# bempt/uda_aerial_semantic_segmentation_research

Measured on AMD Instinct MI355X. Metric: training images/sec at 512x512, higher is better.
Workload: dtype fp32

## Files before the change

include/udaseg.h:

```cpp
#ifndef UDASEG_H
#define UDASEG_H

#include <stddef.h>
#include <stdint.h>

#ifdef __cplusplus
extern "C" {
#endif

#define UDASEG_OK 0
#define UDASEG_E_BADARG (-1)
#define UDASEG_E_UNSUPPORTED (-2)
#define UDASEG_E_WORKSPACE (-3)
#define UDASEG_E_HIP (-4)

#define UDASEG_ACT_NONE 0
#define UDASEG_ACT_LEAKY 1

int udaseg_version(void);
#define UDASEG_OPT_GENERIC_GATHER 0
#define UDASEG_OPT_F32_SPLIT 1
#define UDASEG_OPT_WGRAD_GENERIC 2
#define UDASEG_OPT_F32_HALO 3
#define UDASEG_OPT_F3_CFG 4
#define UDASEG_OPT_F3_WS 5
#define UDASEG_OPT_F3_SIGNS 6
#define UDASEG_OPT_IGEMM_TILE 7
#define UDASEG_OPT_IGEMM_X3 8
#define UDASEG_OPT_NO_FOLD 9
#define UDASEG_OPT_WGRAD_X3_BLOCKS 10
#define UDASEG_OPT_WGRAD_BLOCKS 11
#define UDASEG_OPT_WGRAD_NO_XCD 12
#define UDASEG_OPT_WGRAD_X3 13
#define UDASEG_OPT_NO_WGRAD_HALO 14
#define UDASEG_OPT_WGRAD_F3_BLOCKS 15
#define UDASEG_OPT_WGRAD_HALO_BLOCKS 16
#define UDASEG_OPT_WGRAD_DEEP_BLOCKS 17
#define UDASEG_OPT_WGRAD_DB 18
#define UDASEG_OPT_REDUCE_BLOCKS 19
#define UDASEG_OPT_BN_APPLY_PT 20
#define UDASEG_OPT_GEMM_1X1_TILE 21
#define UDASEG_OPT_GEMM_1X1 22
#define UDASEG_OPT_GEMM_1X1_MAXM 23
#define UDASEG_OPT_NO_STREAM 24
#define UDASEG_OPT_HALO_CFG 25
#define UDASEG_OPT_NO_HALO 26
#define UDASEG_OPT_NO_HALO_S2 27
#define UDASEG_OPT_HALO_W16 28
#define UDASEG_OPT_HALO_DEEP 29
#define UDASEG_OPT_HALO_S2_CK 30
#define UDASEG_OPT_UP_CFG 31
#define UDASEG_OPT_WGRAD_UP_BLOCKS 32
#define UDASEG_OPT_COUNT 33
int udaseg_set_option(int key, int value);
int udaseg_get_option(int key);
int udaseg_option_count(void);
const char* udaseg_option_name(int key);
int udaseg_option_epoch(void);
const char* udaseg_last_error(void);
int udaseg_device_count(void);
int udaseg_memset_async(void* ptr, int value, size_t bytes, void* stream);
int udaseg_stream_wait(void* waiter_stream, void* signal_stream);

typedef struct {
  int n, hi, wi, ci;
  int ho, wo, co;
  int kh, kw, stride, pad;
} udaseg_conv_desc;


int udaseg_conv2d_fwd(const udaseg_conv_desc* d, const float* x, const float* w, const float* bias, float* y,
                      int act, float slope, int accumulate, void* stream);
int udaseg_conv2d_fwd_bnstats(const udaseg_conv_desc* d, const float* x, const float* w, const float* bias, float* y,
                              double* stats, void* stream);
int udaseg_conv2d_fwd_fused(const udaseg_conv_desc* d, const float* x, const float* w, const float* bias,
                            const float* residual, float* y, int act, float slope, void* stream);
int udaseg_conv2d_fwd_bf16(const udaseg_conv_desc* d, const void* x, const void* w, const float* bias, const void* residual,
                           void* y, int out_f32, int act, float slope, double* stats, void* stream);
int udaseg_conv2d_dgrad_bf16(const udaseg_conv_desc* d, const void* dy, const void* w_t, void* dx, int accumulate,
                             void* stream);
int udaseg_conv2d_wgrad_bf16(const udaseg_conv_desc* d, const void* x, const void* dy, float* dw, int accumulate, void* stream);
int udaseg_conv2d_dgrad(const udaseg_conv_desc* d, const float* dy, const float* w_t, float* dx, int accumulate,
                        void* stream);
int udaseg_conv2d_dgrad_bnreduce_ok(const udaseg_conv_desc* d);
int udaseg_conv2d_dgrad_bnreduce(const udaseg_conv_desc* d, const float* dy, const float* w_t, float* dx, const float* prev_y,
                                 const float* save_mean, const float* save_rstd, const float* gamma, const float* beta, int act,
                                 float slope, double* bsums, void* stream);
int udaseg_conv2d_dgrad_bnreduce_bf16_ok(const udaseg_conv_desc* d);
int udaseg_conv2d_dgrad_bnreduce_bf16(const udaseg_conv_desc* d, const void* dy, const void* w_t, void* dx, const void* prev_y,
                                      const float* save_mean, const float* save_rstd, const float* gamma, const float* beta,
                                      int act, float slope, double* bsums, void* stream);
int udaseg_conv2d_wgrad(const udaseg_conv_desc* d, const float* x, const float* dy, float* dw, int accumulate,
                        void* stream);
int udaseg_conv2d_fwd_upcat(const udaseg_conv_desc* d, const float* a, const float* skip, int ca, const float* w,
                            const float* bias, float* y, int act, float slope, double* stats, void* stream);
int udaseg_conv2d_fwd_upcat_bf16(const udaseg_conv_desc* d, const void* a, const void* skip, int ca, const void* w,
                                 const float* bias, void* y, int act, float slope, double* stats, void* stream);
int udaseg_conv2d_dgrad_split(const udaseg_conv_desc* d, const float* dy, const float* w_t, float* dx_a, float* dx_b, int ca,
                              void* stream);
int udaseg_conv2d_dgrad_split_bf16(const udaseg_conv_desc* d, const void* dy, const void* w_t, void* dx_a, void* dx_b, int ca,
                                   void* stream);
int udaseg_conv2d_wgrad_part(const udaseg_conv_desc* d, const float* src, int src_c, int c_off, int up, const float* dy,
                             float* dw, int accumulate, void* stream);
int udaseg_conv2d_wgrad_part_bf16(const udaseg_conv_desc* d, const void* src, int src_c, int c_off, int up, const void* dy,
                                  float* dw, int accumulate, void* stream);
int udaseg_pack_dgrad_weights(const udaseg_conv_desc* d, const float* w, float* w_t, void* stream);
// ... 227 lines not shown
```

uda_aerial_semantic_segmentation_research_amd/_lib.py:

```python
import ctypes as C
import os

_HERE = os.path.dirname(os.path.abspath(__file__))
LIB_PATH = os.environ.get("UDASEG_LIB", os.path.join(_HERE, "libudaseg_hip.so"))

ACT_NONE = 0
ACT_LEAKY = 1


class ConvDesc(C.Structure):
    _fields_ = [(k, C.c_int) for k in ("n", "hi", "wi", "ci", "ho", "wo", "co", "kh", "kw", "stride", "pad")]


_P = C.c_void_p
_I = C.c_int
_L = C.c_int64
_F = C.c_float
_D = C.POINTER(ConvDesc)

SIGNATURES = {
    "udaseg_version": (_I, []),
    "udaseg_set_option": (_I, [_I, _I]),
    "udaseg_get_option": (_I, [_I]),
    "udaseg_option_count": (_I, []),
# ... 92 lines not shown
    "udaseg_bn_bwd_apply_recompute_bf16": (_I, [_P, _P, _P, _P, _P, _P, _P, _P, _P, _P, _P, _L, _I, _I, _F, _P]),
    "udaseg_conv2d_wgrad_halo_bf16_ok": (_I, [_D, _I]),
    "udaseg_conv2d_wgrad_halo_bf16": (_I, [_D, _P, _P, _I, _P, _P, _P]),
    "udaseg_conv2d_wgrad_bnin_bf16": (_I, [_D, _P, _P, _P, _I, _F, _P, _P, _I, _P]),
    "udaseg_frag_elems": (_L, [_I, _I, _I]),
    "udaseg_set_stats_scratch": (_I, [_P, C.c_size_t]),
    "udaseg_pack_frag_batched_bf16": (_I, [_P, _P, _P, _P, _I, _P]),
    "udaseg_conv_frag_ok": (_I, [_D, _I, _I]),
    "udaseg_conv_frag_preferred": (_I, [_D, _I, _I]),
    "udaseg_conv2d_fwd_frag_bf16": (_I, [_D, _P, _P, _I, _P, _P, _P, _P, _I, _F, _P, _I, _I, _F, _P, _P]),
    "udaseg_conv2d_dgrad_frag_bf16": (_I, [_D, _P, _P, _P, _P, _I, _P, _P, _P, _P, _P, _I, _F, _P, _I, _P]),
    "udaseg_pack_frag_batched_f32x3": (_I, [_P, _P, _P, _P, _I, _P]),
    "udaseg_conv2d_wgrad_halo_f32x3_ok": (_I, [_D, _I]),
    "udaseg_conv2d_wgrad_halo_f32x3": (_I, [_D, _P, _P, _I, _P, _P, _P]),
    "udaseg_conv_f32x3_ok": (_I, [_D, _I, _I]),
    "udaseg_f32x3_force_config": (_I, [_I]),
    "udaseg_conv_f32x3_preferred": (_I, [_D, _I, _I]),
    "udaseg_conv2d_fwd_f32x3": (_I, [_D, _P, _P, _I, _P, _P, _P, _I, _F, _P, _P]),
    "udaseg_conv2d_fwd_f32x3_bnin_ok": (_I, [_D, _I]),
    "udaseg_conv2d_fwd_f32x3_bnin_writes": (_I, [_D]),
    "udaseg_conv2d_fwd_f32x3_bnin": (_I, [_D, _P, _I, _P, _P, _I, _F, _P, _P, _P, _P, _I, _F, _P, _P]),
    "udaseg_conv2d_wgrad_bnin_ok": (_I, [_D, _I]),
    "udaseg_conv2d_wgrad_bnin": (_I, [_D, _P, _I, _P, _P, _I, _F, _P, _P, _I, _P]),
    "udaseg_conv2d_dgrad_f32x3": (_I, [_D, _P, _P, _P, _P, _I, _P, _P, _P, _P, _P, _I, _F, _P, _I, _P]),
    "udaseg_conv_up_f32x3_ok": (_I, [_D, _I]),
    "udaseg_pack_up_batched_f32x3": (_I, [_P, _P, _P, _P, _I, _P]),
    "udaseg_conv2d_fwd_up_f32x3": (_I, [_D, _P, _I, _P, _P, _I, _P, _P]),
    "udaseg_conv2d_dgrad_up_f32x3": (_I, [_D, _P, _I, _P, _P, _P, _P, _P, _P, _P, _I, _F, _P, _I, _P]),
    "udaseg_up_f32x3_force_config": (_I, [_I]),
    "udaseg_conv2d_wgrad_up_f32x3_ok": (_I, [_D, _I]),
    "udaseg_conv2d_wgrad_up_f32x3": (_I, [_D, _P, _I, _P, _P, _P]),
    "udaseg_conv2d_wgrad_halo_slice_f32x3": (_I, [_D, _P, _P, _P, _I, _I, _P]),
    "udaseg_wgrad_up_set_blocks": (_I, [_I]),
    "udaseg_conv_stem_f32x3_ok": (_I, [_D]),
    "udaseg_conv2d_fwd_stem_f32x3": (_I, [_D, _P, _P, _P, _P, _P]),
    "udaseg_conv_n16_f32x3_ok": (_I, [_D, _I]),
    "udaseg_conv2d_fwd_n16_f32x3": (_I, [_D, _P, _P, _P, _I, _F, _P, _P, _P, _P]),
    "udaseg_conv2d_dgrad_n16_f32x3": (_I, [_D, _P, _P, _P, _P, _P, _P, _P, _P, _I, _F, _P, _P]),
    "udaseg_set_workspace": (_I, [_P, C.c_size_t]),
    "udaseg_workspace_bytes": (C.c_size_t, [_D]),
    "udaseg_debug_set_timeline": (_I, [_P, _I]),
    "udaseg_fill_f32": (_I, [_P, _L, _F, _P]),
    "udaseg_axpy_f32": (_I, [_P, _P, _L, _F, _P]),
    "udaseg_add_i64": (_I, [_P, _L, _L, _P]),
    "udaseg_prof_enable": (_I, [_I]),
    "udaseg_prof_reset": (_I, []),
    "udaseg_prof_read": (_I, [_I, C.POINTER(C.c_double), C.POINTER(C.c_double), C.POINTER(C.c_int64)]),
    "udaseg_prof_kernel_count": (_I, []),
    "udaseg_prof_kernel_name": (C.c_char_p, [_I]),
    "udaseg_prof_kernel_read": (_I, [_I, C.POINTER(C.c_double), C.POINTER(C.c_double), C.POINTER(C.c_int64)]),
    "udaseg_prof_records": (_I, [_I, _I, C.POINTER(C.c_double), C.POINTER(C.c_double), C.POINTER(C.c_int), C.POINTER(C.c_int)]),
}

OPTIONS = {"GENERIC_GATHER": 0, "F32_SPLIT": 1, "WGRAD_GENERIC": 2, "F32_HALO": 3, "F3_CFG": 4, "F3_WS": 5, "F3_SIGNS": 6, "IGEMM_TILE": 7, "IGEMM_X3": 8, "NO_FOLD": 9, "WGRAD_X3_BLOCKS": 10, "WGRAD_BLOCKS": 11, "WGRAD_NO_XCD": 12, "WGRAD_X3": 13, "NO_WGRAD_HALO": 14, "WGRAD_F3_BLOCKS": 15, "WGRAD_HALO_BLOCKS": 16, "WGRAD_DEEP_BLOCKS": 17, "WGRAD_DB": 18, "REDUCE_BLOCKS": 19, "BN_APPLY_PT": 20, "GEMM_1X1_TILE": 21, "GEMM_1X1": 22, "GEMM_1X1_MAXM": 23, "NO_STREAM": 24, "HALO_CFG": 25, "NO_HALO": 26, "NO_HALO_S2": 27, "HALO_W16": 28, "HALO_DEEP": 29, "HALO_S2_CK": 30, "UP_CFG": 31, "WGRAD_UP_BLOCKS": 32}

_lib = None


def load():
    global _lib
    if _lib is not None:
        return _lib
    if not os.path.exists(LIB_PATH):
        raise RuntimeError(
            f"{LIB_PATH} not found: the HIP extension is not built. Run `python -c \"import __graft_entry__ as g; "
            f"g.build()\"` (or `make -C {os.path.join(_HERE, 'csrc')}`). There is no CPU fallback.")
    lib = C.CDLL(LIB_PATH)
    for name, (res, args) in SIGNATURES.items():
        fn = getattr(lib, name)
        fn.restype = res
        fn.argtypes = args
    _lib = lib
    return lib


def check(rc, what=""):
    if rc != 0:
        msg = load().udaseg_last_error().decode(errors="replace")
        raise RuntimeError(f"libudaseg_hip {what} failed (rc={rc}): {msg}")


def require_gpu():
    lib = load()
    if lib.udaseg_device_count() < 1:
        raise RuntimeError("libudaseg_hip: no HIP device visible; this path has no CPU fallback")
    return lib
```

uda_aerial_semantic_segmentation_research_amd/csrc/api.hip:

```cpp
#include <string.h>
#include <mutex>
#include <vector>

#include "common.h"
#include "options.h"

namespace udaseg {

static thread_local char g_err[512] = "";

void set_error(const char* fmt, ...) {
  va_list ap;
  va_start(ap, fmt);
  vsnprintf(g_err, sizeof(g_err), fmt, ap);
  va_end(ap);
}

int hip_fail(hipError_t e, const char* what) {
  set_error("%s: %s", what, hipGetErrorString(e));
  return UDASEG_E_HIP;
}

struct ProfRec {
  hipEvent_t a, b;
// ... 191 lines not shown
    if (e != hipSuccess) return hip_fail(e, "hipEventSynchronize(prof)");
    float t = 0.f;
    e = hipEventElapsedTime(&t, r.a, r.b);
    if (e != hipSuccess) return hip_fail(e, "hipEventElapsedTime(prof)");
    ms[n] = t;
    flops[n] = r.flops;
    kind[n] = r.kind;
    const int v[11] = {r.d.n, r.d.hi, r.d.wi, r.d.ci, r.d.ho, r.d.wo, r.d.co, r.d.kh, r.d.kw, r.d.stride, r.d.pad};
    for (int i = 0; i < 11; ++i) desc11[n * 11 + i] = v[i];
    ++n;
  }
  return n;
}

namespace udaseg {
enum { K_INT, K_FLAG, K_OFF0 };
struct OptRow {
  const char* env;
  int kind, dflt;
};
static const OptRow g_opt_rows[UDASEG_OPT_COUNT] = {
     {"UDASEG_IGEMM_GENERIC", K_INT, 0},
     {"UDASEG_F32_SPLIT", K_OFF0, 1},
     {"UDASEG_WGRAD_GENERIC", K_INT, 0},
     {"UDASEG_F32_SPLIT", K_OFF0, 1},
     {"UDASEG_F3_CFG", K_INT, 0},
     {"UDASEG_F3_WS", K_OFF0, 1},
     {"UDASEG_F3_SIGNS", K_OFF0, 1},
     {"UDASEG_IGEMM_TILE", K_INT, 0},
     {"UDASEG_IGEMM_X3", K_INT, 1},
     {"UDASEG_NO_FOLD", K_FLAG, 0},
     {"UDASEG_WGRAD_X3_BLOCKS", K_INT, 1024},
     {"UDASEG_WGRAD_BLOCKS", K_INT, 0},
     {"UDASEG_WGRAD_NO_XCD", K_FLAG, 0},
     {"UDASEG_WGRAD_X3", K_OFF0, 1},
     {"UDASEG_NO_WGRAD_HALO", K_FLAG, 0},
     {"UDASEG_WGRAD_F3_BLOCKS", K_INT, 120},
     {"UDASEG_WGRAD_HALO_BLOCKS", K_INT, 96},
     {"UDASEG_WGRAD_DEEP_BLOCKS", K_INT, 0},
     {"UDASEG_WGRAD_DB", K_INT, 1},
     {"UDASEG_REDUCE_BLOCKS", K_INT, 0},
     {"UDASEG_BN_APPLY_PT", K_INT, 4},
     {"UDASEG_GEMM_1X1_TILE", K_INT, 0},
     {"UDASEG_GEMM_1X1", K_OFF0, 1},
     {"UDASEG_GEMM_1X1_MAXM", K_INT, 73728},
     {"UDASEG_NO_STREAM", K_FLAG, 0},
     {"UDASEG_HALO_CFG", K_INT, 0},
     {"UDASEG_NO_HALO", K_FLAG, 0},
     {"UDASEG_NO_HALO_S2", K_FLAG, 0},
     {"UDASEG_HALO_W16", K_INT, 6},
     {"UDASEG_HALO_DEEP", K_OFF0, 1},
     {"UDASEG_HALO_S2_CK", K_INT, 64},
     {"UDASEG_UP_CFG", K_INT, 0},
     {"UDASEG_WGRAD_UP_BLOCKS", K_INT, 0}};
int g_opt_val[UDASEG_OPT_COUNT];
static int g_opt_default[UDASEG_OPT_COUNT];
std::atomic<bool> g_opt_ready{false};
static std::atomic<int> g_opt_epoch{0};
static std::mutex g_opt_mutex;
void opt_init() {
  std::lock_guard<std::mutex> lk(g_opt_mutex);
  if (g_opt_ready.load(std::memory_order_relaxed)) return;
  for (int k = 0; k < UDASEG_OPT_COUNT; ++k) {
    const OptRow& r = g_opt_rows[k];
    const char* e = getenv(r.env);
    int v = r.dflt;
    if (r.kind == K_INT) v = e ? atoi(e) : r.dflt;
    else if (r.kind == K_FLAG) v = e != nullptr ? 1 : 0;
    else v = (e && atoi(e) == 0) ? 0 : 1;
    g_opt_default[k] = g_opt_val[k] = v;
  }
  g_opt_ready.store(true, std::memory_order_release);
}
}

extern "C" int udaseg_set_option(int key, int value) {
  UDASEG_CHECK_ARG(key >= 0 && key < UDASEG_OPT_COUNT, "set_option: unknown key %d (0 .. %d)", key, UDASEG_OPT_COUNT - 1);
  UDASEG_CHECK_ARG(value >= -1, "set_option: value must be >= 0, or -1 for the default");
  udaseg::opt_get(key);
  std::lock_guard<std::mutex> lk(udaseg::g_opt_mutex);
  udaseg::g_opt_val[key] = value < 0 ? udaseg::g_opt_default[key] : value;
  if (key == UDASEG_OPT_GENERIC_GATHER)
    udaseg::g_opt_val[UDASEG_OPT_WGRAD_GENERIC] = value < 0 ? udaseg::g_opt_default[UDASEG_OPT_WGRAD_GENERIC] : value;
  udaseg::g_opt_epoch.fetch_add(1);
  return UDASEG_OK;
}

extern "C" int udaseg_get_option(int key) {
  if (key < 0 || key >= UDASEG_OPT_COUNT) return -1;
  return udaseg::opt_get(key);
}

extern "C" int udaseg_option_count(void) { return UDASEG_OPT_COUNT; }
extern "C" const char* udaseg_option_name(int key) { return key >= 0 && key < UDASEG_OPT_COUNT ? udaseg::g_opt_rows[key].env : ""; }
extern "C" int udaseg_option_epoch(void) { return udaseg::g_opt_epoch.load(); }

extern "C" int udaseg_prof_kernel_count(void) { return g_nkernels; }
extern "C" const char* udaseg_prof_kernel_name(int kid) { return kname(kid); }

extern "C" int udaseg_prof_kernel_read(int kid, double* total_ms, double* total_flops, int64_t* launches) {
  UDASEG_CHECK_ARG(kid >= 0 && kid < g_nkernels && total_ms && total_flops && launches, "prof_kernel_read: bad arguments");
  double ms = 0.0, fl = 0.0;
  for (auto& r : g_krecs[kid]) {
    hipError_t e = hipEventSynchronize(r.b);
    if (e != hipSuccess) return hip_fail(e, "hipEventSynchronize(kprof)");
    float t = 0.f;
    e = hipEventElapsedTime(&t, r.a, r.b);
// ... 10 lines not shown
```

uda_aerial_semantic_segmentation_research_amd/csrc/common.h:

```cpp
#pragma once
#include <stdlib.h>
#include <hip/hip_runtime.h>
#include <stdint.h>
#include <stdio.h>
#include <stdarg.h>
#include <atomic>

#include "../../include/udaseg.h"
#include "options.h"

namespace udaseg {

void set_error(const char* fmt, ...);
int hip_fail(hipError_t e, const char* what);

#define UDASEG_CHECK_ARG(cond, ...)                 \
  do {                                              \
    if (!(cond)) {                                  \
      ::udaseg::set_error(__VA_ARGS__);             \
      return UDASEG_E_BADARG;                       \
    }                                               \
  } while (0)

#define UDASEG_LAUNCH_CHECK(what)                          \
// ... 110 lines not shown
void* workspace_ptr(size_t* bytes);

constexpr int CHSUM_REPLICAS = 16;
constexpr int CHSUM_DIRECT_BLOCKS = 32;
static __global__ void fold_replicas_kernel(const float* __restrict__ rep, int c, float* __restrict__ out, int accumulate) {
  const int i = blockIdx.x * blockDim.x + threadIdx.x;
  if (i >= c) return;
  float s = 0.f;
#pragma unroll
  for (int r = 0; r < CHSUM_REPLICAS; ++r) s += rep[(size_t)r * c + i];
  out[i] = accumulate ? out[i] + s : s;
}

struct StreamShape {
  int bs;
  int grid;
  int c4;
};

static inline StreamShape stream_shape(int64_t n4, int c4, int max_blocks = 2048, int per_thread = 4) {
  StreamShape s;
  s.c4 = c4;
  int unit;
  if (c4 <= 256) {
    s.bs = (256 / c4) * c4;
    unit = 1;
  } else {
    s.bs = 256;
    unit = (c4 + 255) / 256;
    while ((unit * 256) % c4 != 0) ++unit;
  }
  int64_t want = (n4 + (int64_t)s.bs * per_thread - 1) / ((int64_t)s.bs * per_thread);
  if (want > max_blocks) want = max_blocks;
  if (want < 1) want = 1;
  s.grid = (int)(((want + unit - 1) / unit) * unit);
  while ((int64_t)s.grid * s.bs < c4) s.grid += unit;
  return s;
}


static inline int apply_per_thread() {
  const int v = opt_get(UDASEG_OPT_BN_APPLY_PT);
  return (v < 1 || v > 256) ? 4 : v;
}

bool small_conv_applicable(int k, int stride, int pad, int ci_gather, int co_out);
int launch_small_conv(const float* x, const float* w, const float* bias, float* y, int n, int h, int wd, int ci, int co,
                      int flip, int accumulate, int act, float slope, double* stats, const float* residual, hipStream_t s,
                      int up = 0);
bool small_wgrad_applicable(int k, int stride, int pad, int ci, int co, int ntiles);
int launch_small_wgrad(const float* x, const float* dy, float* dw, int n, int h, int wd, int ci, int co, int accumulate,
                       hipStream_t s, int up = 0, const float* in_scale = nullptr, const float* in_shift = nullptr,
                       int in_act = 0, float in_slope = 0.f);

constexpr int PROF_NKERNELS = 24;
int kprof_id(const char* rocprof_symbol);
hipEvent_t kprof_begin(hipStream_t s);
void kprof_end(int kid, hipEvent_t a, hipStream_t s, double flops);
struct KTimer {
  std::atomic<int>* kid;
  hipStream_t s;
  hipEvent_t ev;
  double work;
  KTimer(std::atomic<int>* k, const char* rocprof_symbol, hipStream_t st, double w) : kid(k), s(st), work(w) {
    if (*kid < 0) *kid = kprof_id(rocprof_symbol);
    ev = kprof_begin(s);
  }
  ~KTimer() { kprof_end(*kid, ev, s, work); }
};
void prof_begin(int family, hipStream_t s);
void prof_suspend(int on);
void prof_end(int family, hipStream_t s, double flops, int kind, const udaseg_conv_desc* d);

}
```

uda_aerial_semantic_segmentation_research_amd/csrc/conv_small.hip:

```cpp
#include "common.h"

namespace udaseg {

constexpr int ST = 16;
constexpr int SH = ST + 2;

constexpr int MAX_DEVICES = 16;
static void* g_workspace[MAX_DEVICES] = {};
static size_t g_workspace_bytes[MAX_DEVICES] = {};
static int current_device() {
  int dev = 0;
  if (hipGetDevice(&dev) != hipSuccess || dev < 0 || dev >= MAX_DEVICES) return -1;
  return dev;
}

struct SmallArgs {
  const float* x;
  const float* w;
  const float* bias;
  float* y;
  int n, h, wd, ci, co;
  const float* residual;
  double* stats;
  int flip;
// ... 418 lines not shown
    hipLaunchKernelGGL((conv3x3_small_kernel<2, 1>), dim3(small_grid(a.ntiles, 3)), block, 0, s, a);
    kprof_end(5, ev, s, fl);
  } else if (G == 1 && T == 2) {
    hipLaunchKernelGGL((conv3x3_small_kernel<1, 2>), dim3(small_grid(a.ntiles, 6)), block, 0, s, a);
    kprof_end(6, ev, s, fl);
  } else {
    set_error("small conv: unsupported channel groups G=%d T=%d", G, T);
    return UDASEG_E_UNSUPPORTED;
  }
  UDASEG_LAUNCH_CHECK("conv3x3_small launch");
  return UDASEG_OK;
}

bool small_wgrad_applicable(int k, int stride, int pad, int ci, int co, int ntiles) {
  if (!small_conv_applicable(k, stride, pad, ci, co)) return false;
  const int G = (ci + 15) / 16, T = (co + 15) / 16;
  const size_t need = (size_t)small_grid(ntiles, 2) * (16 * T) * 9 * (16 * G) * sizeof(float);
  const int dev = current_device();
  return dev >= 0 && g_workspace[dev] != nullptr && g_workspace_bytes[dev] >= need;
}

int launch_small_wgrad(const float* x, const float* dy, float* dw, int n, int h, int wd, int ci, int co, int accumulate,
                       hipStream_t s, int up, const float* in_scale, const float* in_shift, int in_act, float in_slope) {
  SmallWgradArgs a = {};
  a.up = up;
  a.in_scale = in_scale; a.in_shift = in_shift; a.in_act = in_act; a.in_slope = in_slope;
  const int dev = current_device();
  if (dev < 0 || g_workspace[dev] == nullptr) {
    set_error("small wgrad: no workspace bound to the current device");
    return UDASEG_E_WORKSPACE;
  }
  a.x = x; a.dy = dy; a.partial = static_cast<float*>(g_workspace[dev]);
  a.n = n; a.h = h; a.w = wd; a.ci = ci; a.co = co;
  a.tiles_x = cdiv(wd, ST); a.tiles_y = cdiv(h, ST); a.ntiles = n * a.tiles_x * a.tiles_y;
  const int G = cdiv(ci, 16), T = cdiv(co, 16);
  const int grid = small_grid(a.ntiles, 2);
  dim3 block(256);
  const double fl = 2.0 * (double)n * h * wd * co * 9.0 * ci;
  hipEvent_t ev = kprof_begin(s);
  if (G == 1 && T == 1) {
    hipLaunchKernelGGL((conv3x3_small_wgrad_kernel<1, 1>), dim3(grid), block, 0, s, a);
    kprof_end(9, ev, s, fl);
  } else if (G == 2 && T == 1) {
    hipLaunchKernelGGL((conv3x3_small_wgrad_kernel<2, 1>), dim3(grid), block, 0, s, a);
    kprof_end(10, ev, s, fl);
  } else if (G == 1 && T == 2) {
    hipLaunchKernelGGL((conv3x3_small_wgrad_kernel<1, 2>), dim3(grid), block, 0, s, a);
    kprof_end(11, ev, s, fl);
  } else {
    set_error("small wgrad: unsupported channel groups G=%d T=%d", G, T);
    return UDASEG_E_UNSUPPORTED;
  }
  UDASEG_LAUNCH_CHECK("conv3x3_small_wgrad launch");
  const int out = 16 * T * 9 * 16 * G;
  if (!accumulate) {
    hipError_t e = hipMemsetAsync(dw, 0, (size_t)co * 9 * ci * sizeof(float), s);
    if (e != hipSuccess) return hip_fail(e, "hipMemsetAsync(small wgrad)");
  }
  hipLaunchKernelGGL(small_wgrad_fold_kernel, dim3(cdiv(out, 256), FOLD_SLICES), dim3(256), 0, s, a.partial, grid, 16 * T, 16 * G,
                     co, ci, dw);
  UDASEG_LAUNCH_CHECK("small_wgrad_fold launch");
  return UDASEG_OK;
}

}

namespace udaseg {
void* workspace_ptr(size_t* bytes) {
  const int dev = current_device();
  if (dev < 0 || g_workspace[dev] == nullptr) {
    if (bytes) *bytes = 0;
    return nullptr;
  }
  if (bytes) *bytes = g_workspace_bytes[dev];
  return g_workspace[dev];
}
}

extern "C" size_t udaseg_workspace_bytes(const udaseg_conv_desc* d) {
  if (!d || d->kh != d->kw || !udaseg::small_conv_applicable(d->kh, d->stride, d->pad, d->ci, d->co)) return 0;
  const int G = (d->ci + 15) / 16, T = (d->co + 15) / 16;
  const int ntiles = d->n * udaseg::cdiv(d->hi, udaseg::ST) * udaseg::cdiv(d->wi, udaseg::ST);
  return (size_t)udaseg::small_grid(ntiles, 2) * (16 * T) * 9 * (16 * G) * sizeof(float);
}

extern "C" int udaseg_set_workspace(void* ptr, size_t bytes) {
  const int dev = udaseg::current_device();
  UDASEG_CHECK_ARG(dev >= 0, "set_workspace: no current HIP device (or more than %d devices)", udaseg::MAX_DEVICES);
  udaseg::g_workspace[dev] = ptr;
  udaseg::g_workspace_bytes[dev] = ptr ? bytes : 0;
  return UDASEG_OK;
}
```

uda_aerial_semantic_segmentation_research_amd/csrc/conv_wgrad.hip:

```cpp
#include <stdlib.h>

#include <type_traits>

#include "common.h"
#include "halo_common.h"

namespace udaseg {

struct WgradArgs {
  const void* x;
  const void* dy;
  float* dw;
  int hi, wi, ci, ho, wo, co;
  int kw, stride, pad;
  int M, J;
  int kchunk;
  int use_atomic;
  float inv_ci, inv_kw, inv_wo, inv_ho;
  int row_uniform;
  unsigned x_bytes, dy_bytes;
  int ci_full, c_off, J_ld, up;
  const float* in_scale;
  const float* in_shift;
  int in_act;
// ... 866 lines not shown
}


}

using namespace udaseg;

static bool wgrad_x3_on() {
  return udaseg::opt_get(UDASEG_OPT_WGRAD_X3) != 0 && udaseg::f32_split_enabled();
}

static int conv2d_wgrad_impl(const udaseg_conv_desc* d, const void* x, int src_c, int c_off, int up, const void* dy, float* dw,
                             int accumulate, void* stream, int bf16, const float* in_scale = nullptr, const float* in_shift = nullptr,
                             int in_act = UDASEG_ACT_NONE, float in_slope = 0.f) {
  UDASEG_CHECK_ARG(d && x && dy && dw, "conv2d_wgrad: NULL pointer");
  const int g = bf16 ? 8 : 4;
  UDASEG_CHECK_ARG(d->ci % g == 0 && d->co % g == 0 && d->ci > 0 && d->co > 0, "conv2d_wgrad: channels must be multiples of %d", g);
  UDASEG_CHECK_ARG(d->kh > 0 && d->kw > 0 && d->stride >= 1 && d->pad >= 0, "conv2d_wgrad: bad kernel/stride");
  UDASEG_CHECK_ARG(d->n > 0 && d->hi > 0 && d->wi > 0 && d->ho > 0 && d->wo > 0, "conv2d_wgrad: non-positive extent");
  UDASEG_CHECK_ARG(d->ho == (d->hi + 2 * d->pad - d->kh) / d->stride + 1 && d->wo == (d->wi + 2 * d->pad - d->kw) / d->stride + 1,
                   "conv2d_wgrad: output extent %dx%d inconsistent with input %dx%d k%d s%d p%d", d->ho, d->wo, d->hi, d->wi,
                   d->kh, d->stride, d->pad);
  UDASEG_CHECK_ARG((long long)d->n * d->hi * d->wi * d->ci < (1LL << 31) && (long long)d->n * d->ho * d->wo * d->co < (1LL << 31),
                   "conv2d_wgrad: tensor exceeds 2^31 elements");
  UDASEG_CHECK_ARG(src_c > 0 && src_c % g == 0 && c_off >= 0 && c_off % g == 0 && c_off + src_c <= d->ci,
                   "conv2d_wgrad_part: channel slice [%d, %d) of %d", c_off, c_off + src_c, d->ci);
  UDASEG_CHECK_ARG(!up || (d->stride == 1 && d->hi % 2 == 0 && d->wi % 2 == 0), "conv2d_wgrad_part: an up-sampled source needs stride 1 and even extents");
  const bool whole = src_c == d->ci;
  UDASEG_CHECK_ARG(whole || accumulate, "conv2d_wgrad_part: a channel slice of dW must be accumulated onto a caller-zeroed gradient");
  WgradArgs a = {};
  a.x = x; a.dy = dy; a.dw = dw;
  a.hi = d->hi; a.wi = d->wi; a.ci = src_c; a.ho = d->ho; a.wo = d->wo; a.co = d->co;
  a.kw = d->kw; a.stride = d->stride; a.pad = d->pad;
  a.M = d->n * d->ho * d->wo;
  a.J = d->kh * d->kw * src_c;
  a.ci_full = d->ci; a.c_off = c_off; a.J_ld = d->kh * d->kw * d->ci; a.up = up;
  a.in_scale = in_scale; a.in_shift = in_shift; a.in_act = in_act; a.in_slope = in_slope;
  a.inv_ci = 1.0f / src_c; a.inv_kw = 1.0f / d->kw; a.inv_wo = 1.0f / d->wo; a.inv_ho = 1.0f / d->ho;
  if (d->kh == 1 && d->kw == 1 && d->stride == 1 && d->pad == 0 && !up) {
    a.hi = 1; a.wi = a.M; a.ho = 1; a.wo = a.M;
    a.inv_wo = 1.0f / (float)a.M; a.inv_ho = 1.0f;
  }
  hipStream_t st = as_stream(stream);
  prof_begin(1, st);
  int rc;
  udaseg_conv_desc dp = *d;
  dp.ci = src_c;
  if (bf16)
    rc = d->co >= 128 ? launch_wgrad<128, 64, 2, 2>(a, accumulate, st, true)
       : d->co > 32   ? launch_wgrad<64, 64, 2, 2>(a, accumulate, st, true)
                      : launch_wgrad<32, 128, 1, 4>(a, accumulate, st, true);
  else if (whole && d->kh == d->kw &&
           small_wgrad_applicable(d->kh, d->stride, d->pad, d->ci, d->co, d->n * cdiv(d->hi, 16) * cdiv(d->wi, 16)))
    rc = launch_small_wgrad(static_cast<const float*>(x), static_cast<const float*>(dy), dw, d->n, d->hi, d->wi, d->ci, d->co,
                            accumulate, st, up);
  else if (d->co > 32 && src_c % 8 == 0 && d->co % 8 == 0 && wgrad_x3_on()) rc = launch_wgrad_x3<64, 64, 2, 2>(a, accumulate, st);
  else if (d->co > 32) rc = launch_wgrad<64, 64, 2, 2>(a, accumulate, st);
  else rc = launch_wgrad<32, 128, 1, 4>(a, accumulate, st);
  prof_end(1, st, udaseg_conv_flops(&dp), 2, &dp);
  return rc;
}

extern "C" int udaseg_conv2d_wgrad(const udaseg_conv_desc* d, const float* x, const float* dy, float* dw,
                                   int accumulate, void* stream) {
  UDASEG_CHECK_ARG(d != nullptr, "conv2d_wgrad: NULL desc");
  return conv2d_wgrad_impl(d, x, d->ci, 0, 0, dy, dw, accumulate, stream, 0);
}

extern "C" int udaseg_conv2d_wgrad_bf16(const udaseg_conv_desc* d, const void* x, const void* dy, float* dw, int accumulate,
                                        void* stream) {
  UDASEG_CHECK_ARG(d != nullptr, "conv2d_wgrad_bf16: NULL desc");
  return conv2d_wgrad_impl(d, x, d->ci, 0, 0, dy, dw, accumulate, stream, 1);
}

extern "C" int udaseg_conv2d_wgrad_bnin_bf16(const udaseg_conv_desc* d, const void* x, const float* in_scale, const float* in_shift,
                                             int in_act, float in_slope, const void* dy, float* dw, int accumulate, void* stream) {
  UDASEG_CHECK_ARG(d != nullptr && in_scale != nullptr && in_shift != nullptr, "conv2d_wgrad_bnin_bf16: NULL desc / scale / shift");
  return conv2d_wgrad_impl(d, x, d->ci, 0, 0, dy, dw, accumulate, stream, 1, in_scale, in_shift, in_act, in_slope);
}

namespace udaseg {
bool wgrad_h2_applicable(const udaseg_conv_desc* d, int up_ca, bool f32);
int launch_wgrad_h2(const udaseg_conv_desc* d, const void* x, const void* x2, int up_ca, const void* dy, float* dw, bool f32, hipStream_t s,
                    const float* in_scale = nullptr, const float* in_shift = nullptr, int in_act = 0, float in_slope = 0.f,
                    int ldw = 0, int dw_coff = 0);
static bool wgrad_halo_off(bool f32) {
  const bool off = opt_get(UDASEG_OPT_NO_WGRAD_HALO) != 0;
  return f32 ? (off || !f32_halo_enabled()) : off;
}
}

extern "C" int udaseg_conv2d_wgrad_bnin_ok(const udaseg_conv_desc* d, int up) {
  if (!d || d->kh != 3 || d->kw != 3 || d->stride != 1 || d->pad != 1 || d->n <= 0 || d->hi <= 0 || d->wi <= 0 || d->ci % 8 != 0 ||
      d->co % 4 != 0)
    return 0;
  if (small_wgrad_applicable(d->kh, d->stride, d->pad, d->ci, d->co, d->n * cdiv(d->hi, 16) * cdiv(d->wi, 16))) return 1;
  return !up && !wgrad_halo_off(true) && wgrad_h2_applicable(d, 0, true) ? 1 : 0;
}

extern "C" int udaseg_conv2d_wgrad_bnin(const udaseg_conv_desc* d, const float* x, int up, const float* in_scale, const float* in_shift,
                                        int in_act, float in_slope, const float* dy, float* dw, int accumulate, void* stream) {
  UDASEG_CHECK_ARG(d && x && in_scale && in_shift && dy && dw, "conv2d_wgrad_bnin: NULL pointer");
  UDASEG_CHECK_ARG(in_act == UDASEG_ACT_NONE || in_act == UDASEG_ACT_LEAKY, "conv2d_wgrad_bnin: unknown activation %d", in_act);
  UDASEG_CHECK_ARG(d->ho == d->hi && d->wo == d->wi, "conv2d_wgrad_bnin: stride-1 'same' convolutions only");
  UDASEG_CHECK_ARG(!up || (d->hi % 2 == 0 && d->wi % 2 == 0), "conv2d_wgrad_bnin: an up-sampled source needs even extents");
  if (!udaseg_conv2d_wgrad_bnin_ok(d, up)) {
    set_error("conv2d_wgrad_bnin: geometry not supported (ask udaseg_conv2d_wgrad_bnin_ok)");
    return UDASEG_E_UNSUPPORTED;
  }
  hipStream_t st = as_stream(stream);
  const bool small = small_wgrad_applicable(d->kh, d->stride, d->pad, d->ci, d->co, d->n * cdiv(d->hi, 16) * cdiv(d->wi, 16));
  if (!small && !accumulate) {
    hipError_t e = hipMemsetAsync(dw, 0, (size_t)d->co * 9 * d->ci * sizeof(float), st);
    if (e != hipSuccess) return hip_fail(e, "hipMemsetAsync(dw)");
  }
  prof_begin(1, st);
  int rc;
  if (small) {
    rc = launch_small_wgrad(x, dy, dw, d->n, d->hi, d->wi, d->ci, d->co, accumulate, st, up, in_scale, in_shift, in_act, in_slope);
  } else {
    rc = launch_wgrad_h2(d, x, nullptr, 0, dy, dw, true, st, in_scale, in_shift, in_act, in_slope);
  }
  prof_end(1, st, udaseg_conv_flops(d), 2, d);
  return rc;
}

extern "C" int udaseg_conv2d_wgrad_halo_bf16_ok(const udaseg_conv_desc* d, int up_ca) {
  return d != nullptr && !wgrad_halo_off(false) && wgrad_h2_applicable(d, up_ca, false) ? 1 : 0;
}

extern "C" int udaseg_conv2d_wgrad_halo_bf16(const udaseg_conv_desc* d, const void* x, const void* skip, int up_ca, const void* dy,
                                             float* dw, void* stream) {
  UDASEG_CHECK_ARG(d && x && dy && dw, "conv2d_wgrad_halo_bf16: NULL pointer");
  UDASEG_CHECK_ARG(d->n > 0 && d->hi > 0 && d->wi > 0 && d->ho == d->hi && d->wo == d->wi, "conv2d_wgrad_halo_bf16: bad extents");
  UDASEG_CHECK_ARG(up_ca == 0 ? skip == nullptr : skip != nullptr, "conv2d_wgrad_halo_bf16: up_ca and skip come together");
  if (!udaseg_conv2d_wgrad_halo_bf16_ok(d, up_ca)) {
    set_error("conv2d_wgrad_halo_bf16: geometry not supported (ask udaseg_conv2d_wgrad_halo_bf16_ok first)");
    return UDASEG_E_UNSUPPORTED;
  }
  hipStream_t st = as_stream(stream);
  prof_begin(1, st);
  const int rc = launch_wgrad_h2(d, x, skip, up_ca, dy, dw, false, st);
  prof_end(1, st, udaseg_conv_flops(d), 2, d);
  return rc;
}

extern "C" int udaseg_conv2d_wgrad_halo_f32x3_ok(const udaseg_conv_desc* d, int up_ca) {
  return d != nullptr && !wgrad_halo_off(true) && wgrad_h2_applicable(d, up_ca, true) ? 1 : 0;
}

extern "C" int udaseg_conv2d_wgrad_halo_f32x3(const udaseg_conv_desc* d, const float* x, const float* skip, int up_ca, const float* dy,
                                              float* dw, void* stream) {
  UDASEG_CHECK_ARG(d && x && dy && dw, "conv2d_wgrad_halo_f32x3: NULL pointer");
  UDASEG_CHECK_ARG(d->n > 0 && d->hi > 0 && d->wi > 0 && d->ho == d->hi && d->wo == d->wi, "conv2d_wgrad_halo_f32x3: bad extents");
  UDASEG_CHECK_ARG((up_ca > 0) == (skip != nullptr), "conv2d_wgrad_halo_f32x3: up_ca=%d, skip %s", up_ca, skip ? "given" : "NULL");
  if (!udaseg_conv2d_wgrad_halo_f32x3_ok(d, up_ca)) {
    set_error("conv2d_wgrad_halo_f32x3: geometry not supported (ask udaseg_conv2d_wgrad_halo_f32x3_ok first)");
    return UDASEG_E_UNSUPPORTED;
  }
  hipStream_t st = as_stream(stream);
  prof_begin(1, st);
  const int rc = launch_wgrad_h2(d, x, skip, up_ca, dy, dw, true, st);
  prof_end(1, st, udaseg_conv_flops(d), 2, d);
  return rc;
}

extern "C" int udaseg_conv2d_wgrad_halo_slice_f32x3(const udaseg_conv_desc* d, const float* x, const float* dy, float* dw, int ldw,
                                                    int c_off, void* stream) {
  UDASEG_CHECK_ARG(d && x && dy && dw, "conv2d_wgrad_halo_slice_f32x3: NULL pointer");
  UDASEG_CHECK_ARG(d->n > 0 && d->hi > 0 && d->wi > 0 && d->ho == d->hi && d->wo == d->wi, "conv2d_wgrad_halo_slice_f32x3: bad extents");
  UDASEG_CHECK_ARG(ldw >= d->ci && c_off >= 0 && c_off + d->ci <= ldw && c_off % 4 == 0 && ldw % 4 == 0,
// ... 75 lines not shown
```

Before: 1069.

## Add persistent bf16x3 MFMA weight-gradient kernel for small-channel 3x3 convs

Adds a new persistent weight-gradient kernel for 3x3 stride-1 convolutions with at most 32 input and output channels. It stages x and dy tiles in LDS as three bf16 pieces that together emulate fp32, reads them with transposing LDS loads, and accumulates with 16x16x32 bf16 MFMA. Each block writes a per-block partial that the existing fold kernel then reduces. It replaces the small-wgrad path by default, and alternates signs across tiles, which may affect rounding behaviour.

Result: faster. 1093 (median of 6 runs) (+2.2%).

```diff
diff --git a/include/udaseg.h b/include/udaseg.h
--- a/include/udaseg.h
+++ b/include/udaseg.h
@@ -51,7 +51,9 @@
 #define UDASEG_OPT_HALO_S2_CK 30
 #define UDASEG_OPT_UP_CFG 31
 #define UDASEG_OPT_WGRAD_UP_BLOCKS 32
-#define UDASEG_OPT_COUNT 33
+#define UDASEG_OPT_WGRAD_N16 33
+#define UDASEG_OPT_WGRAD_N16_BLOCKS 34
+#define UDASEG_OPT_COUNT 35
 int udaseg_set_option(int key, int value);
 int udaseg_get_option(int key);
 int udaseg_option_count(void);
diff --git a/uda_aerial_semantic_segmentation_research_amd/_lib.py b/uda_aerial_semantic_segmentation_research_amd/_lib.py
--- a/uda_aerial_semantic_segmentation_research_amd/_lib.py
+++ b/uda_aerial_semantic_segmentation_research_amd/_lib.py
@@ -168,7 +168,7 @@
     "udaseg_prof_records": (_I, [_I, _I, C.POINTER(C.c_double), C.POINTER(C.c_double), C.POINTER(C.c_int), C.POINTER(C.c_int)]),
 }
 
-OPTIONS = {"GENERIC_GATHER": 0, "F32_SPLIT": 1, "WGRAD_GENERIC": 2, "F32_HALO": 3, "F3_CFG": 4, "F3_WS": 5, "F3_SIGNS": 6, "IGEMM_TILE": 7, "IGEMM_X3": 8, "NO_FOLD": 9, "WGRAD_X3_BLOCKS": 10, "WGRAD_BLOCKS": 11, "WGRAD_NO_XCD": 12, "WGRAD_X3": 13, "NO_WGRAD_HALO": 14, "WGRAD_F3_BLOCKS": 15, "WGRAD_HALO_BLOCKS": 16, "WGRAD_DEEP_BLOCKS": 17, "WGRAD_DB": 18, "REDUCE_BLOCKS": 19, "BN_APPLY_PT": 20, "GEMM_1X1_TILE": 21, "GEMM_1X1": 22, "GEMM_1X1_MAXM": 23, "NO_STREAM": 24, "HALO_CFG": 25, "NO_HALO": 26, "NO_HALO_S2": 27, "HALO_W16": 28, "HALO_DEEP": 29, "HALO_S2_CK": 30, "UP_CFG": 31, "WGRAD_UP_BLOCKS": 32}
+OPTIONS = {"GENERIC_GATHER": 0, "F32_SPLIT": 1, "WGRAD_GENERIC": 2, "F32_HALO": 3, "F3_CFG": 4, "F3_WS": 5, "F3_SIGNS": 6, "IGEMM_TILE": 7, "IGEMM_X3": 8, "NO_FOLD": 9, "WGRAD_X3_BLOCKS": 10, "WGRAD_BLOCKS": 11, "WGRAD_NO_XCD": 12, "WGRAD_X3": 13, "NO_WGRAD_HALO": 14, "WGRAD_F3_BLOCKS": 15, "WGRAD_HALO_BLOCKS": 16, "WGRAD_DEEP_BLOCKS": 17, "WGRAD_DB": 18, "REDUCE_BLOCKS": 19, "BN_APPLY_PT": 20, "GEMM_1X1_TILE": 21, "GEMM_1X1": 22, "GEMM_1X1_MAXM": 23, "NO_STREAM": 24, "HALO_CFG": 25, "NO_HALO": 26, "NO_HALO_S2": 27, "HALO_W16": 28, "HALO_DEEP": 29, "HALO_S2_CK": 30, "UP_CFG": 31, "WGRAD_UP_BLOCKS": 32, "WGRAD_N16": 33, "WGRAD_N16_BLOCKS": 34}
 
 _lib = None
 
diff --git a/uda_aerial_semantic_segmentation_research_amd/csrc/api.hip b/uda_aerial_semantic_segmentation_research_amd/csrc/api.hip
--- a/uda_aerial_semantic_segmentation_research_amd/csrc/api.hip
+++ b/uda_aerial_semantic_segmentation_research_amd/csrc/api.hip
@@ -267,7 +267,9 @@
      {"UDASEG_HALO_DEEP", K_OFF0, 1},
      {"UDASEG_HALO_S2_CK", K_INT, 64},
      {"UDASEG_UP_CFG", K_INT, 0},
-     {"UDASEG_WGRAD_UP_BLOCKS", K_INT, 0}};
+     {"UDASEG_WGRAD_UP_BLOCKS", K_INT, 0},
+     {"UDASEG_WGRAD_N16", K_OFF0, 1},
+     {"UDASEG_WGRAD_N16_BLOCKS", K_INT, 0}};
 int g_opt_val[UDASEG_OPT_COUNT];
 static int g_opt_default[UDASEG_OPT_COUNT];
 std::atomic<bool> g_opt_ready{false};
diff --git a/uda_aerial_semantic_segmentation_research_amd/csrc/common.h b/uda_aerial_semantic_segmentation_research_amd/csrc/common.h
--- a/uda_aerial_semantic_segmentation_research_amd/csrc/common.h
+++ b/uda_aerial_semantic_segmentation_research_amd/csrc/common.h
@@ -186,6 +186,11 @@
 int launch_small_wgrad(const float* x, const float* dy, float* dw, int n, int h, int wd, int ci, int co, int accumulate,
                        hipStream_t s, int up = 0, const float* in_scale = nullptr, const float* in_shift = nullptr,
                        int in_act = 0, float in_slope = 0.f);
+int small_wgrad_fold(const float* partial, int nblocks, int cop, int cip, int co, int ci, float* dw, int accumulate, hipStream_t s);
+bool wgrad_n16_applicable(int k, int stride, int pad, int n, int h, int w, int ci, int co);
+int launch_wgrad_n16(const float* x, const float* dy, float* dw, int n, int h, int wd, int ci, int co, int accumulate,
+                     hipStream_t s, int up = 0, const float* in_scale = nullptr, const float* in_shift = nullptr,
+                     int in_act = 0, float in_slope = 0.f);
 
 constexpr int PROF_NKERNELS = 24;
 int kprof_id(const char* rocprof_symbol);
diff --git a/uda_aerial_semantic_segmentation_research_amd/csrc/conv_small.hip b/uda_aerial_semantic_segmentation_research_amd/csrc/conv_small.hip
--- a/uda_aerial_semantic_segmentation_research_amd/csrc/conv_small.hip
+++ b/uda_aerial_semantic_segmentation_research_amd/csrc/conv_small.hip
@@ -494,13 +494,16 @@
     return UDASEG_E_UNSUPPORTED;
   }
   UDASEG_LAUNCH_CHECK("conv3x3_small_wgrad launch");
-  const int out = 16 * T * 9 * 16 * G;
+  return small_wgrad_fold(a.partial, grid, 16 * T, 16 * G, co, ci, dw, accumulate, s);
+}
+
+int small_wgrad_fold(const float* partial, int nblocks, int cop, int cip, int co, int ci, float* dw, int accumulate, hipStream_t s) {
+  const int out = cop * 9 * cip;
   if (!accumulate) {
     hipError_t e = hipMemsetAsync(dw, 0, (size_t)co * 9 * ci * sizeof(float), s);
     if (e != hipSuccess) return hip_fail(e, "hipMemsetAsync(small wgrad)");
   }
-  hipLaunchKernelGGL(small_wgrad_fold_kernel, dim3(cdiv(out, 256), FOLD_SLICES), dim3(256), 0, s, a.partial, grid, 16 * T, 16 * G,
-                     co, ci, dw);
+  hipLaunchKernelGGL(small_wgrad_fold_kernel, dim3(cdiv(out, 256), FOLD_SLICES), dim3(256), 0, s, partial, nblocks, cop, cip, co, ci, dw);
   UDASEG_LAUNCH_CHECK("small_wgrad_fold launch");
   return UDASEG_OK;
 }
diff --git a/uda_aerial_semantic_segmentation_research_amd/csrc/conv_wgrad.hip b/uda_aerial_semantic_segmentation_research_amd/csrc/conv_wgrad.hip
--- a/uda_aerial_semantic_segmentation_research_amd/csrc/conv_wgrad.hip
+++ b/uda_aerial_semantic_segmentation_research_amd/csrc/conv_wgrad.hip
@@ -942,8 +942,11 @@
                       : launch_wgrad<32, 128, 1, 4>(a, accumulate, st, true);
   else if (whole && d->kh == d->kw &&
            small_wgrad_applicable(d->kh, d->stride, d->pad, d->ci, d->co, d->n * cdiv(d->hi, 16) * cdiv(d->wi, 16)))
-    rc = launch_small_wgrad(static_cast<const float*>(x), static_cast<const float*>(dy), dw, d->n, d->hi, d->wi, d->ci, d->co,
-                            accumulate, st, up);
+    rc = wgrad_n16_applicable(d->kh, d->stride, d->pad, d->n, d->hi, d->wi, d->ci, d->co)
+             ? launch_wgrad_n16(static_cast<const float*>(x), static_cast<const float*>(dy), dw, d->n, d->hi, d->wi, d->ci, d->co,
+                                accumulate, st, up)
+             : launch_small_wgrad(static_cast<const float*>(x), static_cast<const float*>(dy), dw, d->n, d->hi, d->wi, d->ci, d->co,
+                                  accumulate, st, up);
   else if (d->co > 32 && src_c % 8 == 0 && d->co % 8 == 0 && wgrad_x3_on()) rc = launch_wgrad_x3<64, 64, 2, 2>(a, accumulate, st);
   else if (d->co > 32) rc = launch_wgrad<64, 64, 2, 2>(a, accumulate, st);
   else rc = launch_wgrad<32, 128, 1, 4>(a, accumulate, st);
@@ -1006,7 +1009,9 @@
   }
   prof_begin(1, st);
   int rc;
-  if (small) {
+  if (small && wgrad_n16_applicable(d->kh, d->stride, d->pad, d->n, d->hi, d->wi, d->ci, d->co)) {
+    rc = launch_wgrad_n16(x, dy, dw, d->n, d->hi, d->wi, d->ci, d->co, accumulate, st, up, in_scale, in_shift, in_act, in_slope);
+  } else if (small) {
     rc = launch_small_wgrad(x, dy, dw, d->n, d->hi, d->wi, d->ci, d->co, accumulate, st, up, in_scale, in_shift, in_act, in_slope);
   } else {
     rc = launch_wgrad_h2(d, x, nullptr, 0, dy, dw, true, st, in_scale, in_shift, in_act, in_slope);
diff --git a/uda_aerial_semantic_segmentation_research_amd/csrc/conv_wgrad_n16_f32x3.hip b/uda_aerial_semantic_segmentation_research_amd/csrc/conv_wgrad_n16_f32x3.hip
--- /dev/null
+++ b/uda_aerial_semantic_segmentation_research_amd/csrc/conv_wgrad_n16_f32x3.hip
@@ -0,0 +1,290 @@
+#include "common.h"
+#include "halo_common.h"
+
+namespace udaseg {
+
+typedef short n16_s16x4 __attribute__((ext_vector_type(4)));
+typedef short n16_s16x8 __attribute__((ext_vector_type(8)));
+
+struct WgradN16Args {
+  const float* x;
+  const float* dy;
+  float* partial;
+  int n, h, w, ci, co;
+  int ntx, nty, ntiles;
+  unsigned x_bytes, dy_bytes;
+  const float* in_scale;
+  const float* in_shift;
+  int in_act;
+  float in_slope;
+};
+
+constexpr int n16_pad(int bytes) { return (bytes / 64) % 2 == 0 ? bytes + 64 : bytes; }
+
+template <int G_, int T_, int TR_>
+struct WgN16 {
+  static constexpr int G = G_, T = T_, TR = TR_;
+  static constexpr int NT = 256, TW = 32;
+  static constexpr int CIP = 16 * G, COP = 16 * T, NP = G * T;
+  static constexpr int WPP = 4 / NP;
+  static constexpr int RW = TR / WPP;
+  static constexpr int HR = TR + 2, HWD = TW + 2;
+  static constexpr int XSP = n16_pad(HR * HWD * 32), DSP = n16_pad(TR * TW * 32);
+  static constexpr int XPLANE = G * XSP, DPLANE = T * DSP;
+  static constexpr int LDS_TILE = 3 * (XPLANE + DPLANE);
+  static constexpr int OUT = COP * 9 * CIP;
+  static constexpr int LDS = LDS_TILE > OUT * 4 ? LDS_TILE : OUT * 4;
+  static constexpr int XO = CIP / 8, DO = COP / 8;
+  static constexpr int XPC = HR * HWD * XO, DPC = TR * TW * DO;
+  static constexpr int NX = (XPC + NT - 1) / NT, ND = (DPC + NT - 1) / NT;
+  static_assert(NP == 1 || NP == 2, "one or two 16 x 16 pairs");
+  static_assert(TR % WPP == 0, "rows split evenly over a pair's waves");
+  static_assert(NT % XO == 0, "one channel octet per staging thread");
+  static_assert(LDS <= 64 * 1024, "static LDS");
+};
+
+__device__ __forceinline__ bf16x8 n16_fragment(const char* p) {
+  const n16_s16x4 lo = __builtin_amdgcn_ds_read_tr16_b64_v4i16((n16_s16x4 __attribute__((address_space(3)))*)(p));
+  const n16_s16x4 hi = __builtin_amdgcn_ds_read_tr16_b64_v4i16((n16_s16x4 __attribute__((address_space(3)))*)(p + 512));
+  const n16_s16x8 f = __builtin_shufflevector(lo, hi, 0, 1, 2, 3, 4, 5, 6, 7);
+  return __builtin_bit_cast(bf16x8, f);
+}
+
+template <int G, int T, int TR, bool BN, bool UP>
+__global__ __launch_bounds__(256, 2) void conv3x3_n16_f32x3_kernel(const WgradN16Args a) {
+  using C = WgN16<G, T, TR>;
+  __shared__ __attribute__((aligned(16))) char smem[C::LDS];
+  char* const Xs = smem;
+  char* const Ds = smem + 3 * C::XPLANE;
+  const int tid = threadIdx.x, lane = tid & 63;
+  const int wave = __builtin_amdgcn_readfirstlane(tid >> 6);
+  const int pair = wave % C::NP, r0 = (wave / C::NP) * C::RW;
+  const int g = pair % G, ct = pair / G;
+  const int H = a.h, W = a.w;
+
+  __amdgpu_buffer_rsrc_t rs_x = __builtin_amdgcn_make_buffer_rsrc(const_cast<float*>(a.x), 0, (int)a.x_bytes, 0x00020000);
+  __amdgpu_buffer_rsrc_t rs_d = __builtin_amdgcn_make_buffer_rsrc(const_cast<float*>(a.dy), 0, (int)a.dy_bytes, 0x00020000);
+
+  u32x4 sx[C::NX][2], sd[C::ND][2];
+  unsigned x_in = 0;
+  f32x4 xsc[2] = {{0.f, 0.f, 0.f, 0.f}, {0.f, 0.f, 0.f, 0.f}}, xsh[2] = {{0.f, 0.f, 0.f, 0.f}, {0.f, 0.f, 0.f, 0.f}};
+  if constexpr (BN) {
+    const int ch = (tid % C::XO) * 8;
+    if (ch < a.ci) {
+      xsc[0] = *reinterpret_cast<const f32x4*>(a.in_scale + ch);
+      xsc[1] = *reinterpret_cast<const f32x4*>(a.in_scale + ch + 4);
+      xsh[0] = *reinterpret_cast<const f32x4*>(a.in_shift + ch);
+      xsh[1] = *reinterpret_cast<const f32x4*>(a.in_shift + ch + 4);
+    }
+  }
+  auto load_tile = [&](int tile) {
+    const int tx = tile % a.ntx, t2 = tile / a.ntx;
+    const int ty = t2 % a.nty, img = t2 / a.nty;
+    const int y0 = ty * TR, x0 = tx * C::TW;
+    x_in = 0;
+#pragma unroll
+    for (int i = 0; i < C::NX; ++i) {
+      const int pc = tid + i * C::NT;
+      const int pix = pc / C::XO, oct = pc % C::XO;
+      const int hy = pix / C::HWD, hx = pix - hy * C::HWD;
+      const int iy = y0 + hy - 1, ix = x0 + hx - 1;
+      const bool ok = pc < C::XPC && (unsigned)iy < (unsigned)H && (unsigned)ix < (unsigned)W && oct * 8 < a.ci;
+      const int p = UP ? (img * (H >> 1) + (iy >> 1)) * (W >> 1) + (ix >> 1) : (img * H + iy) * W + ix;
+      const unsigned off = ok ? (unsigned)((p * a.ci + oct * 8) * 4) : 0x80000000u;
+      if constexpr (BN) x_in |= (ok ? 1u : 0u) << i;
+      sx[i][0] = __builtin_amdgcn_raw_buffer_load_b128(rs_x, (int)off, 0, 0);
+      sx[i][1] = __builtin_amdgcn_raw_buffer_load_b128(rs_x, (int)off, 16, 0);
+    }
+#pragma unroll
+    for (int i = 0; i < C::ND; ++i) {
+      const int pc = tid + i * C::NT;
+      const int pix = pc / C::DO, oct = pc % C::DO;
+      const int oy = y0 + pix / C::TW, ox = x0 + pix % C::TW;
+      const bool ok = pc < C::DPC && oy < H && ox < W && oct * 8 < a.co;
+      const unsigned off = ok ? (unsigned)((((img * H + oy) * W + ox) * a.co + oct * 8) * 4) : 0x80000000u;
+      sd[i][0] = __builtin_amdgcn_raw_buffer_load_b128(rs_d, (int)off, 0, 0);
+      sd[i][1] = __builtin_amdgcn_raw_buffer_load_b128(rs_d, (int)off, 16, 0);
+    }
+  };
+  auto store_piece = [&](char* dst, int plane_bytes, const u32x4 (&v)[2], unsigned sgn) {
+    u32x4 p0, p1, p2;
+    split3(v[0] ^ sgn, v[1] ^ sgn, p0, p1, p2);
+    *reinterpret_cast<u32x4*>(dst) = p0;
+    *reinterpret_cast<u32x4*>(dst + plane_bytes) = p1;
+    *reinterpret_cast<u32x4*>(dst + 2 * plane_bytes) = p2;
+  };
+  const int P = (int)gridDim.x;
+  auto store_tile = [&](int seq) {
+    const unsigned dsgn = (seq & 1) ? 0x80000000u : 0u;
+#pragma unroll
+    for (int i = 0; i < C::NX; ++i) {
+      const int pc = tid + i * C::NT;
+      const int pix = pc / C::XO, oct = pc % C::XO;
+      if constexpr (BN) {
+        const bool in = (x_in >> i) & 1u;
+#pragma unroll
+        for (int l = 0; l < 2; ++l) {
+          f32x4 v = __builtin_bit_cast(f32x4, sx[i][l]);
+#pragma unroll
+          for (int e = 0; e < 4; ++e) {
+            const float t = act_apply(__builtin_fmaf(v[e], xsc[l][e], xsh[l][e]), a.in_act, a.in_slope);
+            v[e] = in ? t : 0.f;
+          }
+          sx[i][l] = __builtin_bit_cast(u32x4, v);
+        }
+      }
+      if (i < C::NX - 1 || pc < C::XPC) store_piece(Xs + (oct >> 1) * C::XSP + pix * 32 + (oct & 1) * 16, C::XPLANE, sx[i], 0u);
+    }
+#pragma unroll
+    for (int i = 0; i < C::ND; ++i) {
+      const int pc = tid + i * C::NT;
+      const int pix = pc / C::DO, oct = pc % C::DO;
+      if (i < C::ND - 1 || pc < C::DPC) store_piece(Ds + (oct >> 1) * C::DSP + pix * 32 + (oct & 1) * 16, C::DPLANE, sd[i], dsgn);
+    }
+  };
+
+  f32x4 acc[9];
+#pragma unroll
+  for (int t = 0; t < 9; ++t) acc[t] = f32x4{0.f, 0.f, 0.f, 0.f};
+
+  const char* const dbase = Ds + ct * C::DSP + r0 * C::TW * 32 + lane * 8;
+  const char* const xbase = Xs + g * C::XSP + r0 * C::HWD * 32 + lane * 8;
+
+  if ((int)blockIdx.x < a.ntiles) load_tile(blockIdx.x);
+  int seq = 0;
+  for (int tile = blockIdx.x; tile < a.ntiles; tile += P, ++seq) {
+    __syncthreads();
+    store_tile(seq);
+    __syncthreads();
+    if (tile + P < a.ntiles) load_tile(tile + P);
+
+    f32x4 tacc[9];
+#pragma unroll
+    for (int t = 0; t < 9; ++t) tacc[t] = f32x4{0.f, 0.f, 0.f, 0.f};
+    bf16x8 A[3][3];
+#pragma unroll
+    for (int rr = 0; rr < C::RW + 2; ++rr) {
+      if (rr < C::RW) {
+#pragma unroll
+        for (int pl = 0; pl < 3; ++pl) A[rr % 3][pl] = n16_fragment(dbase + pl * C::DPLANE + rr * C::TW * 32);
+      }
+#pragma unroll
+      for (int dx = 0; dx < 3; ++dx) {
+        bf16x8 B[3];
+#pragma unroll
+        for (int pl = 0; pl < 3; ++pl) B[pl] = n16_fragment(xbase + pl * C::XPLANE + (rr * C::HWD + dx) * 32);
+#pragma unroll
+        for (int ky = 0; ky < 3; ++ky) {
+          const int j = rr - ky;
+          if (j >= 0 && j < C::RW) {
+#pragma unroll
+            for (int ij = 2; ij >= 0; --ij)
+#pragma unroll
+              for (int i = 0; i <= ij; ++i)
+                tacc[ky * 3 + dx] = __builtin_amdgcn_mfma_f32_16x16x32_bf16(A[j % 3][i], B[ij - i], tacc[ky * 3 + dx], 0, 0, 0);
+          }
+        }
+      }
+    }
+    if (seq & 1) {
+#pragma unroll
+      for (int t = 0; t < 9; ++t) acc[t] -= tacc[t];
+    } else {
+#pragma unroll
+      for (int t = 0; t < 9; ++t) acc[t] += tacc[t];
+    }
+  }
+
+  float* const out = reinterpret_cast<float*>(smem);
+  __syncthreads();
+  for (int wv = 0; wv < 4; ++wv) {
+    if (wave == wv) {
+#pragma unroll
+      for (int t = 0; t < 9; ++t)
+#pragma unroll
+        for (int v = 0; v < 4; ++v) {
+          const int idx = ((16 * ct + 4 * (lane >> 4) + v) * 9 + t) * C::CIP + 16 * g + (lane & 15);
+          out[idx] = (wv < C::NP ? 0.f : out[idx]) + acc[t][v];
+        }
+    }
+    __syncthreads();
+  }
+  float* const dst = a.partial + (size_t)blockIdx.x * C::OUT;
+  for (int idx = tid; idx < C::OUT; idx += C::NT) dst[idx] = out[idx];
+}
+
+bool wgrad_n16_applicable(int k, int stride, int pad, int n, int h, int w, int ci, int co) {
+  if (opt_get(UDASEG_OPT_WGRAD_N16) == 0 || !f32_halo_enabled()) return false;
+  if (k != 3 || stride != 1 || pad != 1 || n <= 0 || h <= 0 || w <= 0) return false;
+  if (ci <= 0 || co <= 0 || ci % 8 != 0 || co % 8 != 0 || ci > 32 || co > 32) return false;
+  const int G = (ci + 15) / 16, T = (co + 15) / 16;
+  if (G * T > 2) return false;
+  const long long px = (long long)n * h * w;
+  return px * ci * 4 < (1LL << 31) && px * co * 4 < (1LL << 31);
+}
+
+template <int G, int T, int TR, bool BN, bool UP>
+static void launch_n16_t(const WgradN16Args& a, int grid, hipStream_t s) {
+  static std::atomic<int> kid{-1};
+  if (kid < 0) {
+    char nm[96];
+    snprintf(nm, sizeof(nm), "conv3x3_n16_f32x3_kernel<%d, %d, %d, %s, %s>", G, T, TR, BN ? "true" : "false", UP ? "true" : "false");
+    kid = kprof_id(nm);
+  }
+  hipEvent_t ev = kprof_begin(s);
+  hipLaunchKernelGGL((conv3x3_n16_f32x3_kernel<G, T, TR, BN, UP>), dim3(grid), dim3(256), 0, s, a);
+  kprof_end(kid, ev, s, 2.0 * (double)a.n * a.h * a.w * a.co * 9.0 * a.ci);
+}
+
+template <int G, int T, int TR>
+static void launch_n16_forms(const WgradN16Args& a, int grid, hipStream_t s, bool up) {
+  const bool bn = a.in_scale != nullptr;
+  if (bn && up) launch_n16_t<G, T, TR, true, true>(a, grid, s);
+  else if (bn) launch_n16_t<G, T, TR, true, false>(a, grid, s);
+  else if (up) launch_n16_t<G, T, TR, false, true>(a, grid, s);
+  else launch_n16_t<G, T, TR, false, false>(a, grid, s);
+}
+
+int launch_wgrad_n16(const float* x, const float* dy, float* dw, int n, int h, int wd, int ci, int co, int accumulate,
+                     hipStream_t s, int up, const float* in_scale, const float* in_shift, int in_act, float in_slope) {
+  if (!wgrad_n16_applicable(3, 1, 1, n, h, wd, ci, co)) {
+    set_error("wgrad_n16: geometry not supported (ci %d, co %d)", ci, co);
+    return UDASEG_E_UNSUPPORTED;
+  }
+  if (up && (h % 2 != 0 || wd % 2 != 0)) {
+    set_error("wgrad_n16: an up-sampled source needs even extents");
+    return UDASEG_E_UNSUPPORTED;
+  }
+  if (in_scale != nullptr && in_shift == nullptr) {
+    set_error("wgrad_n16: in_scale without in_shift");
+    return UDASEG_E_UNSUPPORTED;
+  }
+  const int G = (ci + 15) / 16, T = (co + 15) / 16;
+  const int TR = G * T == 1 ? 8 : 4;
+  WgradN16Args a = {};
+  a.x = x; a.dy = dy;
+  a.n = n; a.h = h; a.w = wd; a.ci = ci; a.co = co;
+  a.ntx = cdiv(wd, 32); a.nty = cdiv(h, TR); a.ntiles = n * a.ntx * a.nty;
+  const long long px = (long long)n * h * wd;
+  a.x_bytes = (unsigned)(up ? (long long)n * (h / 2) * (wd / 2) * ci * 4 : px * ci * 4);
+  a.dy_bytes = (unsigned)(px * co * 4);
+  a.in_scale = in_scale; a.in_shift = in_shift; a.in_act = in_act; a.in_slope = in_slope;
+  size_t ws_bytes = 0;
+  a.partial = static_cast<float*>(workspace_ptr(&ws_bytes));
+  const size_t out_bytes = (size_t)16 * T * 9 * 16 * G * sizeof(float);
+  int grid = opt_get(UDASEG_OPT_WGRAD_N16_BLOCKS);
+  if (grid < 1) grid = 512;
+  if (grid > a.ntiles) grid = a.ntiles;
+  if ((size_t)grid * out_bytes > ws_bytes) grid = (int)(ws_bytes / out_bytes);
+  if (a.partial == nullptr || grid < 1) {
+    set_error("wgrad_n16: no workspace (or too small a one) bound to the current device");
+    return UDASEG_E_WORKSPACE;
+  }
+  if (G == 1 && T == 1) launch_n16_forms<1, 1, 8>(a, grid, s, up != 0);
+  else if (G == 2) launch_n16_forms<2, 1, 4>(a, grid, s, up != 0);
+  else launch_n16_forms<1, 2, 4>(a, grid, s, up != 0);
+  UDASEG_LAUNCH_CHECK("conv3x3_n16_f32x3 (weight gradient) launch");
+  return small_wgrad_fold(a.partial, grid, 16 * T, 16 * G, co, ci, dw, accumulate, s);
+}
+
+}
```
